# balint256/gr-baz

Measured on AMD Instinct MI355X. Metric: MUSIC-DoA snapshots/s (4 ant, 1024 samp, 3600 bins), higher is better.
Workload: dtype f64; 1 GPU; cfg2 (BASELINE.json configs[1]): m=4 n=2 nsamples=1024 (K=256) resolution=3600, spectrum port wired, 8 streams x 32768 items per GPU per step, device-resident; streams_total=8, items_per_launch_sequence=262144, parallelism=independent streams, s mod 1, no collective, collective_backend_fell_back=False

## Files before the change

gr_baz_amd/csrc/music_kernels.hip.h:

```cpp
#pragma once

#include <hip/hip_runtime.h>
#include <stdint.h>

#include "order_kernels.hip.h"

namespace bazmusic {

typedef double v4f64 __attribute__((ext_vector_type(4)));
typedef float v4f32 __attribute__((ext_vector_type(4)));
typedef uint32_t v4u32 __attribute__((ext_vector_type(4)));
typedef double v2f64 __attribute__((ext_vector_type(2)));

__device__ __forceinline__ void wave_lds_fence()
{
    __builtin_amdgcn_fence(__ATOMIC_RELEASE, "wavefront");
    __builtin_amdgcn_wave_barrier();
    __builtin_amdgcn_fence(__ATOMIC_ACQUIRE, "wavefront");
}

template <int M>
__global__ __launch_bounds__(256) void cov_mfma_kernel(const float* __restrict__ in,
                                                        double2* __restrict__ R,
                                                        uint32_t batch, uint32_t K)
// ... 625 lines not shown
            dloc += d.x * d.x + d.y * d.y;
        }
        const double d2 = group_allsum<GS>(dloc);
        if (!conv && ok) {
            ok = ok2 && (d2 == d2);
#pragma unroll
            for (int c = 0; c < P; ++c) y[c] = yn[c];
            if (ok && d2 <= TOL2) conv = true;
            else if (it >= 2 && d2 > 100.0 * TOL2 && d2 > BAIL2 * d2prev) ok = false;
            d2prev = d2;
        }
        if (__all(conv || !ok || !item_ok)) break;
    }
    if (item_ok && j == 0) redo[item] = conv ? 0 : 1;
    if (!__any(conv && item_ok)) return;

    wave_lds_fence();
#pragma unroll
    for (int c = 0; c < P; ++c) sY[g][c][j] = y[c];
    wave_lds_fence();
    const bool emit = conv && item_ok && row;
    if constexpr (P <= 2) {
        if (emit && Ss) {
#pragma unroll
            for (int cI = 0; cI < P; ++cI) {
                Ss[(size_t)((2 * cI) * 2 * M + 2 * j) * qstride + item] = y[cI].x;
                Ss[(size_t)((2 * cI) * 2 * M + 2 * j + 1) * qstride + item] = y[cI].y;
                Ss[(size_t)((2 * cI + 1) * 2 * M + 2 * j) * qstride + item] = -y[cI].y;
                Ss[(size_t)((2 * cI + 1) * 2 * M + 2 * j + 1) * qstride + item] = y[cI].x;
            }
        }
    }
    if (emit && Qs) {
        for (int l = j; l < M; ++l) {
            double re = 0.0, im = 0.0;
#pragma unroll
            for (int c = 0; c < P; ++c) {
                const double2 vl = sY[g][c][l];
                re += y[c].x * vl.x + y[c].y * vl.y;
                im += y[c].y * vl.x - y[c].x * vl.y;
            }
            re = ((l == j) ? 1.0 : 0.0) - re; im = -im;
            if (l == j) {
                Qs[(size_t)(j * M + j) * qstride + item] = re;
            } else {
                Qs[(size_t)(j * M + l) * qstride + item] = 2.0 * re;
                Qs[(size_t)(l * M + j) * qstride + item] = -2.0 * im;
            }
        }
    }
    if (!Gs) return;
    double2 v[P];
    double tau[P];
    double2 w[P];
#pragma unroll
    for (int c = 0; c < P; ++c) w[c] = y[c];
#pragma unroll
    for (int c = 0; c < P; ++c) {
        const bool in = row && j >= c;
        const double2 x = in ? w[c] : make_double2(0.0, 0.0);
        const double nx2 = group_allsum<GS>(x.x * x.x + x.y * x.y);
        const double xcr = group_allsum<GS>(j == c ? x.x : 0.0), xci = group_allsum<GS>(j == c ? x.y : 0.0);
        const double nx = sqrt(nx2), ax = sqrt(xcr * xcr + xci * xci);
        const double pr = ax > 0.0 ? xcr / ax : 1.0, pi = ax > 0.0 ? xci / ax : 0.0;
        v[c] = x;
        if (j == c) { v[c].x += pr * nx; v[c].y += pi * nx; }
        const double nv2 = group_allsum<GS>(v[c].x * v[c].x + v[c].y * v[c].y);
        tau[c] = nv2 > 0.0 ? 2.0 / nv2 : 0.0;
#pragma unroll
        for (int b = c + 1; b < P; ++b) {
            const double2 t = cmulc(w[b], v[c]);
            const double sr = group_allsum<GS>(t.x) * tau[c], si = group_allsum<GS>(t.y) * tau[c];
            w[b].x -= v[c].x * sr - v[c].y * si;
            w[b].y -= v[c].x * si + v[c].y * sr;
        }
    }
    double2 beta[P][P];
#pragma unroll
    for (int c = 0; c < P; ++c)
#pragma unroll
        for (int c2 = c + 1; c2 < P; ++c2) {
            const double2 t = cmulc(v[c2], v[c]);
            beta[c][c2] = make_double2(group_allsum<GS>(t.x), group_allsum<GS>(t.y));
        }
    wave_lds_fence();
#pragma unroll
    for (int c = 0; c < P; ++c) sY[g][c][j] = v[c];
    wave_lds_fence();
    if (emit) {
        for (int k = P; k < M; ++k) {
            double2 coef[P];
            double2 gk = make_double2(j == k ? 1.0 : 0.0, 0.0);
#pragma unroll
            for (int c = P - 1; c >= 0; --c) {
                const double2 vk = sY[g][c][k];
                double2 s = make_double2(vk.x, -vk.y);
#pragma unroll
                for (int c2 = c + 1; c2 < P; ++c2) {
                    const double2 t = cmul(coef[c2], beta[c][c2]);
                    s.x -= t.x; s.y -= t.y;
                }
                coef[c] = make_double2(tau[c] * s.x, tau[c] * s.y);
                const double2 t = cmul(coef[c], v[c]);
                gk.x -= t.x; gk.y -= t.y;
            }
            const int r = k - P;
            Gs[(size_t)((r * M + j) * 2) * qstride + item] = gk.x;
            Gs[(size_t)((r * M + j) * 2 + 1) * qstride + item] = gk.y;
        }
    }
}

#define BAZ_KEY_EMPTY_BITS 0x7FEFFFFFFFF00000ull

__device__ __forceinline__ double key_empty() { return __builtin_bit_cast(double, (uint64_t)BAZ_KEY_EMPTY_BITS); }

__device__ __forceinline__ double vmin64(double a, double b)
{
    double r;
    asm("v_min_f64 %0, %1, %2" : "=v"(r) : "v"(a), "v"(b));
    return r;
}
__device__ __forceinline__ double vmax64(double a, double b)
{
    double r;
    asm("v_max_f64 %0, %1, %2" : "=v"(r) : "v"(a), "v"(b));
    return r;
}

__device__ __forceinline__ double make_key(const double d, const uint32_t bin, const uint32_t keep_mask)
{
    const uint64_t b = __builtin_bit_cast(uint64_t, d);
    const uint32_t lo = ((uint32_t)b & keep_mask) | bin;
    return __builtin_bit_cast(double, (b & 0xFFFFFFFF00000000ull) | lo);
}

template <int NMAX>
__device__ __forceinline__ void key_insert(double (&t)[NMAX], double k)
{
#pragma unroll
    for (int i = 0; i < NMAX; ++i) {
        const double lo = vmin64(k, t[i]);
        if (i + 1 < NMAX) k = vmax64(k, t[i]);
        t[i] = lo;
    }
}

template <int NMAX>
__device__ __forceinline__ void key_insert_new(double (&t)[NMAX], double k)
{
    double lo, hi = 0.0;
    asm("v_min_f64 %0, |%1|, %2" : "=v"(lo) : "v"(k), "v"(t[0]));
    if constexpr (NMAX > 1) asm("v_max_f64 %0, |%1|, %2" : "=v"(hi) : "v"(k), "v"(t[0]));
    t[0] = lo;
    if constexpr (NMAX > 1) {
        k = hi;
#pragma unroll
        for (int i = 1; i < NMAX; ++i) {
            const double l2 = vmin64(k, t[i]);
            if (i + 1 < NMAX) k = vmax64(k, t[i]);
            t[i] = l2;
        }
    }
}

template <int NMAX>
__device__ __forceinline__ void key_merge_xor(double (&t)[NMAX], const int mask)
{
    double o[NMAX];
#pragma unroll
    for (int i = 0; i < NMAX; ++i) o[i] = __shfl_xor(t[i], mask, 64);
#pragma unroll
    for (int i = 0; i < NMAX; ++i) key_insert<NMAX>(t, o[i]);
}

__device__ __forceinline__ float strength_f32(const double d)
{
    return __builtin_amdgcn_rcpf((float)d);
}

struct ScanRefine {
    const double* Gs;
    const double2* TB;
    double below;
    unsigned long long* count;
    const double* A2;
};

template <int M>
__device__ __forceinline__ uint32_t literal_tile(v4f64 (&acc)[4], const ScanRefine& rf, const v2f64* __restrict__ tbl,
                                             const uint32_t st, const uint32_t itc, const int g,
                                             const uint32_t qstride, const int nn, const uint32_t bin, const uint32_t res,
                                             const bool (&row_ok)[4])
{
    constexpr int KS2 = (2 * M + 3) / 4;
    const double* __restrict__ tb1 = reinterpret_cast<const double*>(tbl + (size_t)st * KS2 * 2 * 64);
    uint32_t cnt = 0;
    if constexpr (KS2 <= 2) {
        constexpr int KMAX = M - 1;
        double x0[KMAX][KS2], x1[KMAX][KS2];
        const double sgn1 = (g & 1) ? 1.0 : -1.0;
        uint32_t itq = itc, gq = (uint32_t)g;
        asm volatile("" : "+v"(itq), "+v"(gq));
#pragma unroll
        for (int k = 0; k < KMAX; ++k) {
            const int kk = k < nn ? k : 0;
#pragma unroll
            for (int s = 0; s < KS2; ++s) {
                const bool in = 4 * s + (int)gq < 2 * M;
                const uint32_t ant = in ? 2u * (uint32_t)s + (gq >> 1) : 0u;
                const double v0 = rf.Gs[(size_t)(((uint32_t)kk * M + ant) * 2u + (gq & 1u)) * qstride + itq];
                const double v1 = rf.Gs[(size_t)(((uint32_t)kk * M + ant) * 2u + ((gq & 1u) ^ 1u)) * qstride + itq];
                x0[k][s] = in ? v0 : 0.0;
                x1[k][s] = in ? sgn1 * v1 : 0.0;
            }
        }
#pragma unroll
        for (int t = 0; t < 4; ++t) {
            bool want = false;
#pragma unroll
            for (int r = 0; r < 4; ++r) want |= (fabs(acc[t][r]) <= rf.below) && (bin + t < res);
            if (!__any(want)) continue;
            double tbv[KS2];
#pragma unroll
            for (int s = 0; s < KS2; ++s) tbv[s] = tb1[(size_t)(t >> 1) * 128 + (t & 1) + (size_t)s * 256];
            v4f64 d = {0, 0, 0, 0};
#pragma unroll
            for (int k = 0; k < KMAX; ++k) {
                if (k < nn) {
                    v4f64 p = {0, 0, 0, 0};
#pragma unroll
                    for (int s = 0; s < KS2; ++s) p = __builtin_amdgcn_mfma_f64_16x16x4f64(x0[k][s], tbv[s], p, 0, 0, 0);
                    d += p * p;
                    p = (v4f64){0, 0, 0, 0};
#pragma unroll
                    for (int s = 0; s < KS2; ++s) p = __builtin_amdgcn_mfma_f64_16x16x4f64(x1[k][s], tbv[s], p, 0, 0, 0);
                    d += p * p;
                }
            }
#pragma unroll
            for (int r = 0; r < 4; ++r) {
                const bool redo = (fabs(acc[t][r]) <= rf.below) && (bin + t < res);
                acc[t][r] = redo ? d[r] : acc[t][r];
                cnt += (redo && row_ok[r]) ? 1u : 0u;
            }
        }
        return cnt;
    }
#pragma unroll
    for (int t = 0; t < 4; ++t) {
        v4f64 d = {0, 0, 0, 0};
        for (int k = 0; k < nn; ++k) {
#pragma unroll
            for (int part = 0; part < 2; ++part) {
                v4f64 p = {0, 0, 0, 0};
                const int comp = part ? ((g & 1) ^ 1) : (g & 1);
                const double sgn = (part && !(g & 1)) ? -1.0 : 1.0;
                const double* __restrict__ ga = rf.Gs + (size_t)((k * M + (g >> 1)) * 2 + comp) * qstride + itc;
                const double* __restrict__ tb = tb1 + (size_t)(t >> 1) * 128 + (t & 1);
                if constexpr (KS2 <= 2) {
#pragma unroll
                    for (int s = 0; s < KS2; ++s) {
                        const double a = (4 * s + g < 2 * M) ? sgn * ga[(size_t)s * 4 * qstride] : 0.0;
                        p = __builtin_amdgcn_mfma_f64_16x16x4f64(a, tb[(size_t)s * 256], p, 0, 0, 0);
                    }
                } else {
#pragma nounroll
                    for (int s = 0; s < KS2; ++s) {
                        const double a = (4 * s + g < 2 * M) ? sgn * ga[(size_t)s * 4 * qstride] : 0.0;
                        p = __builtin_amdgcn_mfma_f64_16x16x4f64(a, tb[(size_t)s * 256], p, 0, 0, 0);
                    }
                }
                d += p * p;
            }
        }
#pragma unroll
        for (int r = 0; r < 4; ++r) {
            const bool redo = (fabs(acc[t][r]) <= rf.below) && (bin + t < res);
            acc[t][r] = redo ? d[r] : acc[t][r];
            cnt += (redo && row_ok[r]) ? 1u : 0u;
        }
        __builtin_amdgcn_sched_barrier(0);
    }
    return cnt;
}

template <int M, int NMAX, bool SPEC, bool VEC4, int ABL = 0, int AUX = (1 | 2 | 16), int SIG = 0>
__global__ __launch_bounds__(256, (M <= 4 && NMAX <= 2) ? ((ABL & 2048) ? 3 : 4) : (M >= 9 ? 2 : 1)) void scan_mfma_kernel(const double* __restrict__ Qs,
                                                         const double2* __restrict__ FB,
                                                         float* __restrict__ spec,
                                                         double* __restrict__ cand,
                                                         uint32_t batch, uint32_t res, uint32_t qstride,
                                                         uint32_t nsplit, uint32_t nclass, uint32_t rows_per_class,
                                                         uint32_t keep_mask, uint32_t n, ScanRefine rf, uint32_t seq_walk = 0)
{
    constexpr int MM = M * M;
    constexpr int KS = SIG ? (2 * M + 3) / 4 : (MM + 3) / 4;
    static_assert(!SIG || (((SIG == 1 && M >= 6) || M >= 9) && KS <= 8), "the short form: one phase per step, no row classes (m >= 6)");
    constexpr int NG = (SIG == 1) ? 2 : 4;
    constexpr int SCH = (KS <= 8) ? KS : 8;
    constexpr int PPS = (KS + SCH - 1) / SCH;
    constexpr int CPP = 2 * SCH;
    constexpr int SPW = (CPP + 3) / 4;
    __shared__ v2f64 stage[2][CPP * 64];

    const int lane = threadIdx.x & 63;
    const int wave = __builtin_amdgcn_readfirstlane(threadIdx.x >> 6);
    const int c = lane & 15, g = lane >> 4;

    const uint32_t split = blockIdx.x % nsplit;
    const uint32_t blk = blockIdx.x / nsplit;
    uint32_t p0;
    if constexpr ((ABL & 4096) == 0) p0 = (blk * 4 + wave) * 16;
    else p0 = (blk % nclass) * rows_per_class + ((blk / nclass) * 4 + wave) * 16;
    const uint32_t cls = __builtin_amdgcn_readfirstlane(p0 / rows_per_class);
    const uint32_t j0 = p0 - cls * rows_per_class;
    const uint32_t sh = ((res & 63u) * cls) & 63u;
    const int shc = (int)(sh >> 2);
    const uint32_t nsteps = (res + sh + 63u) >> 6;
    const uint32_t st_begin = (uint32_t)(((uint64_t)nsteps * split) / nsplit);
    const uint32_t st_end = (uint32_t)(((uint64_t)nsteps * (split + 1)) / nsplit);
    const uint32_t item0 = nclass * j0 + cls;

    double qa[SIG ? 1 : KS];
    [[maybe_unused]] double sa[SIG ? NG : 1][SIG ? KS : 1];
    const uint32_t it_c = item0 + nclass * (uint32_t)c;
    const uint32_t itc = (it_c < batch) ? it_c : (batch - 1);
    if constexpr (SIG) {
#pragma unroll
        for (int q = 0; q < NG; ++q) {
            const int sub = c >> 2;
            const int wrow = (SIG == 1) ? (c & 3) + 4 * (2 * q + (sub >> 1)) : (c & 3) + 4 * q;
            const int outp = (SIG == 1) ? (sub & 1) : sub;
            const uint32_t it_q = item0 + nclass * (uint32_t)wrow;
            const uint32_t itq = (it_q < batch) ? it_q : (batch - 1);
#pragma unroll
            for (int s = 0; s < KS; ++s) {
                const int e = 4 * s + g;
                sa[q][s] = (e < 2 * M) ? Qs[(size_t)(outp * 2 * M + e) * qstride + itq] : 0.0;
            }
        }
        qa[0] = 0.0;
    } else {
#pragma unroll
        for (int s = 0; s < KS; ++s) {
            const int e = 4 * s + g;
            qa[s] = (e < MM) ? Qs[(size_t)e * qstride + itc] : 0.0;
        }
    }

    double key[4][NMAX];
#pragma unroll
    for (int r = 0; r < 4; ++r)
#pragma unroll
        for (int i = 0; i < NMAX; ++i) key[r][i] = key_empty();
    [[maybe_unused]] float gate_f[4];
    [[maybe_unused]] double gate_d[4];
#pragma unroll
    for (int r = 0; r < 4; ++r) {
        gate_f[r] = __builtin_inff();
        gate_d[r] = __builtin_bit_cast(double, (uint64_t)BAZ_KEY_EMPTY_BITS | 0xFFFFFull);
    }
    const bool refine_on = rf.Gs != nullptr;
    uint32_t refined_wave = 0;
    [[maybe_unused]] const float below_f = refine_on ? (float)rf.below : -1.0f;
    [[maybe_unused]] const double below_d = refine_on ? rf.below : -1.0;

    const int cc = c - shc;
    const v2f64* __restrict__ fb = reinterpret_cast<const v2f64*>(FB) + (g * 16 + (cc < 0 ? cc + 16 : cc)) -
                                   (cc < 0 ? KS * 2 * 64 : 0);
    const int wave4 = wave & 3;
    constexpr bool ROT = (ABL & 1024) != 0;
    uint32_t turn = 0;
    v2f64 sreg0 = {0, 0}, sreg1 = {0, 0}, sreg2 = {0, 0}, sreg3 = {0, 0};
    static_assert(SPW <= 4, "a wave stages at most 4 chunks per phase");
#define BAZ_FB_LD(IDX) ((ABL & 256) ? __builtin_nontemporal_load(fb + (IDX)) : fb[(IDX)])
#define BAZ_STAGE_DMA(ST, P, BUF)                                                                \
    do {                                                                                         \
        if (wave4 == (int)(turn & 3u)) {                                                         \
            const int nch__ = 2 * ((KS - (P) * SCH < SCH) ? (KS - (P) * SCH) : SCH);             \
            const size_t ch0__ = ((size_t)(ST) * KS + (size_t)(P) * SCH) * 2;                    \
            _Pragma("unroll")                                                                    \
            for (int j__ = 0; j__ < CPP; ++j__)                                                  \
                if (j__ < nch__)                                                                 \
                    __builtin_amdgcn_global_load_lds((const __attribute__((address_space(1))) void*)(fb + (ch0__ + j__) * 64), \
                                                     (__attribute__((address_space(3))) void*)(&stage[(BUF)][j__ * 64]), 16, 0, 0); \
        }                                                                                        \
    } while (0)
#define BAZ_STAGE_LOAD(ST, P)                                                                    \
    do {                                  \
        if constexpr (!(ABL & 128)) {                                                            \
        const int nch__ = 2 * ((KS - (P) * SCH < SCH) ? (KS - (P) * SCH) : SCH);                 \
        const size_t ch0__ = ((size_t)(ST) * KS + (size_t)(P) * SCH) * 2;                        \
        sreg0 = BAZ_FB_LD((ch0__ + (wave4 < nch__ ? wave4 : nch__ - 1)) * 64);                   \
        if constexpr (SPW > 1) sreg1 = BAZ_FB_LD((ch0__ + (wave4 + 4 < nch__ ? wave4 + 4 : nch__ - 1)) * 64);   \
        if constexpr (SPW > 2) sreg2 = BAZ_FB_LD((ch0__ + (wave4 + 8 < nch__ ? wave4 + 8 : nch__ - 1)) * 64);   \
        if constexpr (SPW > 3) sreg3 = BAZ_FB_LD((ch0__ + (wave4 + 12 < nch__ ? wave4 + 12 : nch__ - 1)) * 64); \
        }                                                                                        \
    } while (0)
#define BAZ_STAGE_STORE(BUF, P)                                                                  \
    do {                                                                                         \
        const int nch__ = 2 * ((KS - (P) * SCH < SCH) ? (KS - (P) * SCH) : SCH);                 \
        if (wave4 < nch__) stage[(BUF)][wave4 * 64 + lane] = sreg0;                              \
        if constexpr (SPW > 1) { if (wave4 + 4 < nch__) stage[(BUF)][(wave4 + 4) * 64 + lane] = sreg1; }   \
        if constexpr (SPW > 2) { if (wave4 + 8 < nch__) stage[(BUF)][(wave4 + 8) * 64 + lane] = sreg2; }   \
        if constexpr (SPW > 3) { if (wave4 + 12 < nch__) stage[(BUF)][(wave4 + 12) * 64 + lane] = sreg3; } \
    } while (0)

    if (st_begin < st_end) {
        if constexpr (ROT) {
            BAZ_STAGE_DMA(st_begin, 0, 0);
            asm volatile("s_waitcnt vmcnt(0)" ::: "memory");
            ++turn;
        } else {
            BAZ_STAGE_LOAD(st_begin, 0);
            BAZ_STAGE_STORE(0, 0);
        }
    }
    __syncthreads();

    int buf = 0;
    v4f32 sv[4] = {{0, 0, 0, 0}, {0, 0, 0, 0}, {0, 0, 0, 0}, {0, 0, 0, 0}};
    float* __restrict__ spec_base = SPEC ? spec + (size_t)item0 * res - sh : nullptr;
    uint32_t soff0 = 0;
    const uint32_t row4 = 4u * nclass * res * 4u;
    [[maybe_unused]] __amdgpu_buffer_rsrc_t spec_rsrc = __builtin_amdgcn_make_buffer_rsrc(spec_base, 0, 0x7FFFFFFF, 0x00020000);
    bool row_ok[4];
#pragma unroll
    for (int r = 0; r < 4; ++r) {
        if (r == 0) soff0 = ((uint32_t)g * nclass * res + 4u * (uint32_t)c) * 4u;
        row_ok[r] = (item0 + nclass * (uint32_t)(g + 4 * r)) < batch;
    }
    const uint32_t nst = st_end - st_begin;
    const uint32_t SW = seq_walk ? 1u : (nst >= 64u ? 8u : (nst >= 16u ? 4u : (nst >= 6u ? 2u : 1u)));
    uint32_t st = st_begin, sweep = 0;
    for (uint32_t it = 0; it < nst; ++it) {
        uint32_t st_next = st + SW, sweep_next = sweep;
        if (st_next >= st_end) { sweep_next = sweep + 1; st_next = st_begin + sweep_next; }
        const bool has_next = it + 1 < nst;
        v4f64 acc[4];
#pragma unroll
        for (int t = 0; t < 4; ++t) acc[t] = (v4f64){0, 0, 0, 0};
        const uint32_t bin = st * 64 + 4 * c - sh;

#pragma unroll
        for (int p = 0; p < PPS; ++p) {
            const bool last_p = (p == PPS - 1);
            const bool more = !last_p || has_next;
            if constexpr (ROT) { if (more) BAZ_STAGE_DMA(last_p ? st_next : st, last_p ? 0 : p + 1, buf ^ 1); }
            else { if (more) BAZ_STAGE_LOAD(last_p ? st_next : st, last_p ? 0 : p + 1); }

            if constexpr (SIG) {
                const v4f64 a2v = *reinterpret_cast<const v4f64*>(rf.A2 + (size_t)st * 64 + 4 * c);
#pragma unroll
                for (int q = 0; q < NG; ++q) {
                    v4f64 tmp[4];
#pragma unroll
                    for (int t = 0; t < 4; ++t) tmp[t] = (v4f64){0, 0, 0, 0};
#pragma unroll
                    for (int sl = 0; sl < KS; ++sl) {
                        const v2f64 f01 = stage[buf][(2 * sl) * 64 + lane];
                        const v2f64 f23 = stage[buf][(2 * sl + 1) * 64 + lane];
                        tmp[0] = __builtin_amdgcn_mfma_f64_16x16x4f64(sa[q][sl], f01.x, tmp[0], 0, 0, 0);
                        tmp[1] = __builtin_amdgcn_mfma_f64_16x16x4f64(sa[q][sl], f01.y, tmp[1], 0, 0, 0);
                        tmp[2] = __builtin_amdgcn_mfma_f64_16x16x4f64(sa[q][sl], f23.x, tmp[2], 0, 0, 0);
                        tmp[3] = __builtin_amdgcn_mfma_f64_16x16x4f64(sa[q][sl], f23.y, tmp[3], 0, 0, 0);
                    }
#pragma unroll
                    for (int t = 0; t < 4; ++t) {
                        if constexpr (SIG == 1) {
                            acc[t][2 * q] = a2v[t] - (tmp[t][0] * tmp[t][0] + tmp[t][1] * tmp[t][1]);
                            acc[t][2 * q + 1] = a2v[t] - (tmp[t][2] * tmp[t][2] + tmp[t][3] * tmp[t][3]);
                        } else {
                            acc[t][q] = a2v[t] - ((tmp[t][0] * tmp[t][0] + tmp[t][1] * tmp[t][1]) +
                                                  (tmp[t][2] * tmp[t][2] + tmp[t][3] * tmp[t][3]));
                        }
                    }
                }
            } else {
            if constexpr (ABL & 8192) __builtin_amdgcn_s_setprio(3);
            if constexpr (ABL & 16384) __builtin_amdgcn_s_setprio(0);
#pragma unroll
            for (int sl = 0; sl < SCH; ++sl) {
                const int s = p * SCH + sl;
                if (s < KS) {
                    const v2f64 f01 = stage[buf][(2 * sl) * 64 + lane];
                    const v2f64 f23 = stage[buf][(2 * sl + 1) * 64 + lane];
                    if constexpr (ABL & 8) {
                        acc[0][s & 3] += qa[s] * f01.x; acc[1][s & 3] += qa[s] * f01.y;
                        acc[2][s & 3] += qa[s] * f23.x; acc[3][s & 3] += qa[s] * f23.y;
                    } else {
                        acc[0] = __builtin_amdgcn_mfma_f64_16x16x4f64(qa[s], f01.x, acc[0], 0, 0, 0);
                        acc[1] = __builtin_amdgcn_mfma_f64_16x16x4f64(qa[s], f01.y, acc[1], 0, 0, 0);
                        acc[2] = __builtin_amdgcn_mfma_f64_16x16x4f64(qa[s], f23.x, acc[2], 0, 0, 0);
                        acc[3] = __builtin_amdgcn_mfma_f64_16x16x4f64(qa[s], f23.y, acc[3], 0, 0, 0);
                    }
                }
            }
            if constexpr (ABL & 8192) __builtin_amdgcn_s_setprio(0);
            if constexpr (ABL & 16384) __builtin_amdgcn_s_setprio(3);
            }

            if (last_p) {
#pragma unroll
                for (int r = 0; r < 4; ++r) asm volatile("" ::"v"(sv[r]));
                bool hit = false, low = false;
#pragma unroll
                for (int r = 0; r < 4; ++r) {
                    if constexpr (SPEC && !(ABL & 4)) {
                        float fd[4];
#pragma unroll
                        for (int t = 0; t < 4; ++t) fd[t] = (float)acc[t][r];
                        if constexpr (!(ABL & 2)) {
                            float mn;
                            asm("v_min3_f32 %0, |%1|, |%2|, |%3|" : "=v"(mn) : "v"(fd[0]), "v"(fd[1]), "v"(fd[2]));
                            asm("v_min_f32 %0, %1, |%2|" : "=v"(mn) : "v"(mn), "v"(fd[3]));
                            hit |= (mn <= gate_f[r]);
                            low |= (mn <= below_f);
                        }
#pragma unroll
                        for (int t = 0; t < 4; ++t) sv[r][t] = __builtin_amdgcn_rcpf(fabsf(fd[t]));
                    } else {
                        if constexpr (!(ABL & 2)) {
                            double m01, m23, mn;
                            asm("v_min_f64 %0, |%1|, |%2|" : "=v"(m01) : "v"(acc[0][r]), "v"(acc[1][r]));
                            asm("v_min_f64 %0, |%1|, |%2|" : "=v"(m23) : "v"(acc[2][r]), "v"(acc[3][r]));
                            mn = vmin64(m01, m23);
                            hit |= (mn <= gate_d[r]);
                            low |= (mn <= below_d);
                        }
                    }
                }
                if constexpr (!(ABL & 2)) {
                    if ((ABL & 64) || __any(hit)) {
                        if (refine_on && __any(low)) {
                            const int cr = c - shc;
                            const v2f64* __restrict__ tbl = reinterpret_cast<const v2f64*>(rf.TB) +
                                (g * 16 + (cr < 0 ? cr + 16 : cr)) - (cr < 0 ? ((2 * M + 3) / 4) * 2 * 64 : 0);
                            uint32_t cnt = literal_tile<M>(acc, rf, tbl, st, itc, g, qstride, (int)M - (int)n, bin, res, row_ok);
                            __builtin_amdgcn_s_waitcnt(0x0F70);
                            if constexpr (SPEC && !(ABL & 4)) {
#pragma unroll
                                for (int r = 0; r < 4; ++r)
#pragma unroll
                                    for (int t = 0; t < 4; ++t) sv[r][t] = strength_f32(fabs(acc[t][r]));
                            }
                            if (rf.count) {
#pragma unroll
                                for (int msk = 1; msk < 64; msk <<= 1) cnt += __shfl_xor(cnt, msk, 64);
                                refined_wave += (uint32_t)__builtin_amdgcn_readfirstlane((int)cnt);
                            }
                        }
                        const uint32_t nobin = ~keep_mask;
#pragma unroll
                        for (int r = 0; r < 4; ++r) {
#pragma unroll
                            for (int t = 0; t < 4; ++t)
                                key_insert_new<NMAX>(key[r], make_key(acc[t][r], (bin + t < res) ? bin + t : nobin, keep_mask));
                            const uint64_t kb = __builtin_bit_cast(uint64_t, key[r][NMAX - 1]) | (uint64_t)(~keep_mask);
                            gate_d[r] = fmax(__builtin_bit_cast(double, kb), below_d);
                            gate_f[r] = (float)gate_d[r];
                        }
                    }
                }
                if constexpr (ABL & 4) {
#pragma unroll
                    for (int r = 0; r < 4; ++r)
#pragma unroll
                        for (int t = 0; t < 4; ++t) sv[r][t] = __builtin_bit_cast(float, (uint32_t)__builtin_bit_cast(uint64_t, acc[t][r]));
                }
            }

            if constexpr (ROT) {
                if (more && wave4 == (int)(turn & 3u)) asm volatile("s_waitcnt vmcnt(0)" ::: "memory");
                if (more) ++turn;
            } else {
                if (more) BAZ_STAGE_STORE(buf ^ 1, last_p ? 0 : p + 1);
            }

            if (last_p) {
                if constexpr (ABL & 1) {
#pragma unroll
                    for (int r = 0; r < 4; ++r) asm volatile("" ::"v"(sv[r]));
                }
                if constexpr (SPEC && !(ABL & 1)) {
                    const int step_off = (int)(st * 256u);
                    if constexpr (VEC4) {
                        if ((st > 0 || sh == 0) && st * 64 + 64 - sh <= res) {
#pragma unroll
                            for (int r = 0; r < 4; ++r)
                                if (row_ok[r]) __builtin_amdgcn_raw_buffer_store_b128(__builtin_bit_cast(v4u32, sv[r]), spec_rsrc, (int)soff0, step_off + (int)(row4 * (uint32_t)r), AUX);
                        } else {
#pragma unroll
                            for (int r = 0; r < 4; ++r)
                                if (row_ok[r] && bin < res) __builtin_amdgcn_raw_buffer_store_b128(__builtin_bit_cast(v4u32, sv[r]), spec_rsrc, (int)soff0, step_off + (int)(row4 * (uint32_t)r), AUX);
                        }
                    } else {
#pragma unroll
                        for (int r = 0; r < 4; ++r) {
                            const v4u32 u = __builtin_bit_cast(v4u32, sv[r]);
#pragma unroll
                            for (int t = 0; t < 4; ++t)
                                if (row_ok[r] && bin + t < res)
                                    __builtin_amdgcn_raw_buffer_store_b32(u[t], spec_rsrc, (int)(soff0 + 4u * t), step_off + (int)(row4 * (uint32_t)r), AUX);
                        }
                    }
                }
            }
            if constexpr (ROT) {
                asm volatile("s_waitcnt lgkmcnt(0)" ::: "memory");
                __builtin_amdgcn_s_barrier();
                asm volatile("" ::: "memory");
            } else {
                __syncthreads();
            }
            buf ^= 1;
        }
        st = st_next;
        sweep = sweep_next;
    }

    if (rf.count && lane == 0 && refined_wave) atomicAdd(rf.count, (unsigned long long)refined_wave);
#pragma unroll
    for (int r = 0; r < 4; ++r) {
        key_merge_xor<NMAX>(key[r], 1);
        key_merge_xor<NMAX>(key[r], 2);
        key_merge_xor<NMAX>(key[r], 4);
        key_merge_xor<NMAX>(key[r], 8);
        const uint32_t it = item0 + nclass * (uint32_t)(g + 4 * r);
        if (c == 0 && it < batch) {
#pragma unroll
            for (int i = 0; i < NMAX; ++i) cand[((size_t)it * nsplit + split) * NMAX + i] = key[r][i];
        }
    }
}

#undef BAZ_STAGE_LOAD
#undef BAZ_STAGE_DMA
#undef BAZ_FB_LD
#undef BAZ_STAGE_STORE

template <int NMAX>
__global__ __launch_bounds__(256) void topn_merge_kernel(const double* __restrict__ cand,
                                                          const float* __restrict__ spec,
                                                          float* __restrict__ ang, float* __restrict__ lvl,
                                                          uint32_t batch, uint32_t res, uint32_t n, uint32_t nsplit,
                                                          uint32_t keep_mask, unsigned long long* __restrict__ next_stat,
                                                          unsigned long long* __restrict__ fire_dev = nullptr,
                                                          unsigned long long* __restrict__ fire_host = nullptr,
                                                          unsigned long long fire_tag = 0ull)
{
    const uint32_t it = blockIdx.x * 256 + threadIdx.x;
    if (it == 0 && next_stat) *next_stat = 0ull;
    if (it == 0 && fire_dev && fire_host) {
        fire_host[0] = fire_dev[0];
        fire_host[1] = fire_dev[1];
        fire_dev[0] = 0ull;
        fire_dev[1] = 0ull;
        __threadfence_system();
        fire_host[2] = fire_tag;
    }
    if (it >= batch) return;
    double key[NMAX];
#pragma unroll
    for (int i = 0; i < NMAX; ++i) key[i] = key_empty();
    const size_t base = (size_t)it * nsplit * NMAX;
    for (uint32_t k = 0; k < nsplit * NMAX; ++k) key_insert<NMAX>(key, cand[base + k]);
#pragma unroll
    for (int i = 0; i < NMAX; ++i)
        if (i < (int)n) {
            const uint64_t b = __builtin_bit_cast(uint64_t, key[i]);
            const uint32_t bin = (uint32_t)b & ~keep_mask;
            const bool used = (b < (uint64_t)BAZ_KEY_EMPTY_BITS) && (bin < res);
            float a = 0.0f, l = 0.0f;
            if (used) {
                a = (float)((double)bin * 360.0 / (double)res);
                if (spec) l = spec[(size_t)it * res + bin];
                else l = strength_f32(__builtin_bit_cast(double, b & ~(uint64_t)(~keep_mask)));
            }
            ang[(size_t)it * n + i] = a;
            if (lvl) lvl[(size_t)it * n + i] = l;
        }
}

template <int NMAX>
__global__ __launch_bounds__(256) void peak_pick_kernel(const float* __restrict__ spec, float* __restrict__ ang,
                                                         float* __restrict__ lvl, uint32_t batch, uint32_t res,
                                                         uint32_t n)
{
    const int lane = threadIdx.x & 63;
    const uint32_t it = blockIdx.x * 4 + (threadIdx.x >> 6);
    if (it >= batch) return;
    const float* __restrict__ s = spec + (size_t)it * res;
    double key[NMAX];
#pragma unroll
    for (int i = 0; i < NMAX; ++i) key[i] = key_empty();
    for (uint32_t b = lane; b < res; b += 64) {
        const float v = s[b];
        const float vp = s[b == 0 ? res - 1 : b - 1];
        const float vn = s[b + 1 == res ? 0 : b + 1];
        if (v > vp && v >= vn && v > 0.0f) {
            const uint64_t k = ((uint64_t)(0x7F800000u - __float_as_uint(v)) << 32) | (uint64_t)b;
            key_insert<NMAX>(key, __builtin_bit_cast(double, k));
        }
    }
#pragma unroll
    for (int mask = 1; mask < 64; mask <<= 1) key_merge_xor<NMAX>(key, mask);
    if (lane == 0) {
#pragma unroll
        for (int i = 0; i < NMAX; ++i)
            if (i < (int)n) {
                const uint64_t k = __builtin_bit_cast(uint64_t, key[i]);
                const bool used = k < (uint64_t)BAZ_KEY_EMPTY_BITS;
                const uint32_t bin = (uint32_t)k;
                ang[(size_t)it * n + i] = used ? (float)((double)bin * 360.0 / (double)res) : 0.0f;
                if (lvl) lvl[(size_t)it * n + i] = used ? __uint_as_float(0x7F800000u - (uint32_t)(k >> 32)) : 0.0f;
            }
    }
}

}
```

Baseline: 230.7 million snapshots/s.

## Software-pipeline spectrum stores behind next step's MFMAs in small-M scan kernel

For the M<=4 single-phase spectrum path, the scan loop now defers each step's spectrum row stores and interleaves them between the next step's MFMA instructions, using sched_barriers to pin the order. The reciprocal and min-gate work for the first two accumulator columns is also moved inside the MFMA sequence so it overlaps matrix issue, and all LDS fragments are loaded up front. The final step's stores are flushed after the loop. This is meant to hide global store and VALU latency behind MFMA work, at the cost of more live registers. The VEC4 fast path now always checks bins per store instead of taking an unchecked full-tile branch.

```diff
diff --git a/gr_baz_amd/csrc/music_kernels.hip.h b/gr_baz_amd/csrc/music_kernels.hip.h
--- a/gr_baz_amd/csrc/music_kernels.hip.h
+++ b/gr_baz_amd/csrc/music_kernels.hip.h
@@ -951,6 +951,7 @@
     constexpr int PPS = (KS + SCH - 1) / SCH;
     constexpr int CPP = 2 * SCH;
     constexpr int SPW = (CPP + 3) / 4;
+    constexpr bool PIPE = !SIG && PPS == 1 && M <= 4 && SPEC && !(ABL & (4 | 8 | 1024));
     __shared__ v2f64 stage[2][CPP * 64];
 
     const int lane = threadIdx.x & 63;
@@ -1080,6 +1081,19 @@
         if (r == 0) soff0 = ((uint32_t)g * nclass * res + 4u * (uint32_t)c) * 4u;
         row_ok[r] = (item0 + nclass * (uint32_t)(g + 4 * r)) < batch;
     }
+    [[maybe_unused]] auto store_row = [&](int r, const v4f32 v, uint32_t st_x, uint32_t bin_x) {
+        const int off = (int)(st_x * 256u + row4 * (uint32_t)r);
+        if constexpr (VEC4) {
+            if (row_ok[r] && bin_x < res) __builtin_amdgcn_raw_buffer_store_b128(__builtin_bit_cast(v4u32, v), spec_rsrc, (int)soff0, off, AUX);
+        } else {
+            const v4u32 u = __builtin_bit_cast(v4u32, v);
+#pragma unroll
+            for (int t = 0; t < 4; ++t)
+                if (row_ok[r] && bin_x + t < res) __builtin_amdgcn_raw_buffer_store_b32(u[t], spec_rsrc, (int)(soff0 + 4u * t), off, AUX);
+        }
+    };
+    constexpr uint32_t NO_BIN = 0x7FFFFFF0u;
+    [[maybe_unused]] uint32_t st_prev = 0, bin_prev = NO_BIN;
     const uint32_t nst = st_end - st_begin;
     const uint32_t SW = seq_walk ? 1u : (nst >= 64u ? 8u : (nst >= 16u ? 4u : (nst >= 6u ? 2u : 1u)));
     uint32_t st = st_begin, sweep = 0;
@@ -1091,6 +1105,7 @@
 #pragma unroll
         for (int t = 0; t < 4; ++t) acc[t] = (v4f64){0, 0, 0, 0};
         const uint32_t bin = st * 64 + 4 * c - sh;
+        [[maybe_unused]] float mn01[4];
 
 #pragma unroll
         for (int p = 0; p < PPS; ++p) {
@@ -1129,6 +1144,40 @@
             } else {
             if constexpr (ABL & 8192) __builtin_amdgcn_s_setprio(3);
             if constexpr (ABL & 16384) __builtin_amdgcn_s_setprio(0);
+            if constexpr (PIPE) {
+                v2f64 f01[KS], f23[KS];
+#pragma unroll
+                for (int s = 0; s < KS; ++s) {
+                    f01[s] = stage[buf][(2 * s) * 64 + lane];
+                    f23[s] = stage[buf][(2 * s + 1) * 64 + lane];
+                }
+                __builtin_amdgcn_sched_barrier(0);
+#pragma unroll
+                for (int s = 0; s < KS; ++s) {
+                    acc[0] = __builtin_amdgcn_mfma_f64_16x16x4f64(qa[s], f01[s].x, acc[0], 0, 0, 0);
+                    acc[1] = __builtin_amdgcn_mfma_f64_16x16x4f64(qa[s], f01[s].y, acc[1], 0, 0, 0);
+                    __builtin_amdgcn_sched_barrier(0);
+                    if constexpr (!(ABL & 1)) {
+#pragma unroll
+                        for (int r = (s * 4) / KS; r < ((s + 1) * 4) / KS; ++r) store_row(r, sv[r], st_prev, bin_prev);
+                        __builtin_amdgcn_sched_barrier(0);
+                    }
+                }
+#pragma unroll
+                for (int s = 0; s < KS; ++s) {
+                    acc[2] = __builtin_amdgcn_mfma_f64_16x16x4f64(qa[s], f23[s].x, acc[2], 0, 0, 0);
+                    acc[3] = __builtin_amdgcn_mfma_f64_16x16x4f64(qa[s], f23[s].y, acc[3], 0, 0, 0);
+                    __builtin_amdgcn_sched_barrier(0);
+#pragma unroll
+                    for (int r = (s * 4) / KS; r < ((s + 1) * 4) / KS; ++r) {
+                        const float f0 = (float)acc[0][r], f1 = (float)acc[1][r];
+                        if constexpr (!(ABL & 2)) asm("v_min_f32 %0, |%1|, |%2|" : "=v"(mn01[r]) : "v"(f0), "v"(f1));
+                        sv[r][0] = __builtin_amdgcn_rcpf(fabsf(f0));
+                        sv[r][1] = __builtin_amdgcn_rcpf(fabsf(f1));
+                    }
+                    __builtin_amdgcn_sched_barrier(0);
+                }
+            } else {
 #pragma unroll
             for (int sl = 0; sl < SCH; ++sl) {
                 const int s = p * SCH + sl;
@@ -1146,17 +1195,30 @@
                     }
                 }
             }
+            }
             if constexpr (ABL & 8192) __builtin_amdgcn_s_setprio(0);
             if constexpr (ABL & 16384) __builtin_amdgcn_s_setprio(3);
             }
 
             if (last_p) {
-#pragma unroll
-                for (int r = 0; r < 4; ++r) asm volatile("" ::"v"(sv[r]));
+                if constexpr (!PIPE) {
+#pragma unroll
+                    for (int r = 0; r < 4; ++r) asm volatile("" ::"v"(sv[r]));
+                }
                 bool hit = false, low = false;
 #pragma unroll
                 for (int r = 0; r < 4; ++r) {
-                    if constexpr (SPEC && !(ABL & 4)) {
+                    if constexpr (PIPE) {
+                        const float f2 = (float)acc[2][r], f3 = (float)acc[3][r];
+                        if constexpr (!(ABL & 2)) {
+                            float mn;
+                            asm("v_min3_f32 %0, %1, |%2|, |%3|" : "=v"(mn) : "v"(mn01[r]), "v"(f2), "v"(f3));
+                            hit |= (mn <= gate_f[r]);
+                            low |= (mn <= below_f);
+                        }
+                        sv[r][2] = __builtin_amdgcn_rcpf(fabsf(f2));
+                        sv[r][3] = __builtin_amdgcn_rcpf(fabsf(f3));
+                    } else if constexpr (SPEC && !(ABL & 4)) {
                         float fd[4];
 #pragma unroll
                         for (int t = 0; t < 4; ++t) fd[t] = (float)acc[t][r];
@@ -1232,28 +1294,12 @@
 #pragma unroll
                     for (int r = 0; r < 4; ++r) asm volatile("" ::"v"(sv[r]));
                 }
-                if constexpr (SPEC && !(ABL & 1)) {
-                    const int step_off = (int)(st * 256u);
-                    if constexpr (VEC4) {
-                        if ((st > 0 || sh == 0) && st * 64 + 64 - sh <= res) {
-#pragma unroll
-                            for (int r = 0; r < 4; ++r)
-                                if (row_ok[r]) __builtin_amdgcn_raw_buffer_store_b128(__builtin_bit_cast(v4u32, sv[r]), spec_rsrc, (int)soff0, step_off + (int)(row4 * (uint32_t)r), AUX);
-                        } else {
-#pragma unroll
-                            for (int r = 0; r < 4; ++r)
-                                if (row_ok[r] && bin < res) __builtin_amdgcn_raw_buffer_store_b128(__builtin_bit_cast(v4u32, sv[r]), spec_rsrc, (int)soff0, step_off + (int)(row4 * (uint32_t)r), AUX);
-                        }
-                    } else {
-#pragma unroll
-                        for (int r = 0; r < 4; ++r) {
-                            const v4u32 u = __builtin_bit_cast(v4u32, sv[r]);
-#pragma unroll
-                            for (int t = 0; t < 4; ++t)
-                                if (row_ok[r] && bin + t < res)
-                                    __builtin_amdgcn_raw_buffer_store_b32(u[t], spec_rsrc, (int)(soff0 + 4u * t), step_off + (int)(row4 * (uint32_t)r), AUX);
-                        }
-                    }
+                if constexpr (PIPE) {
+                    st_prev = st;
+                    bin_prev = bin;
+                } else if constexpr (SPEC && !(ABL & 1)) {
+#pragma unroll
+                    for (int r = 0; r < 4; ++r) store_row(r, sv[r], st, bin);
                 }
             }
             if constexpr (ROT) {
@@ -1267,6 +1313,10 @@
         }
         st = st_next;
         sweep = sweep_next;
+    }
+    if constexpr (PIPE && !(ABL & 1)) {
+#pragma unroll
+        for (int r = 0; r < 4; ++r) store_row(r, sv[r], st_prev, bin_prev);
     }
 
     if (rf.count && lane == 0 && refined_wave) atomicAdd(rf.count, (unsigned long long)refined_wave);
```

New measurement: 229.2 million snapshots/s. No clear change (-0.6%).
